# Rudrabha/Wav2Lip

Hardware: NVIDIA H100
Metric: 96x96 face-crops/sec (B=128, T=5, mel 80x16) (higher is better)
Workload: dtype f16

## Files before the change

wav2lip_b200/csrc/conv_igemm.cuh:

```cuda
#pragma once

#include <cuda.h>
#include <cuda_bf16.h>
#include <cuda_fp16.h>
#include <stdint.h>

#include "wgmma.cuh"

namespace w2l {

constexpr int kTileM = 128;
constexpr int kMaxTaps = 49;
constexpr int kMaxSteps = 3 * kMaxTaps;
constexpr int kSmemExtra = 2048;
constexpr int kSmemMax = 227 * 1024;

enum : int { ACT_NONE = 0, ACT_RELU = 1, ACT_LRELU = 2 };

struct EpiParams {
    int Wout, Hout, N;
    int act;
    int out_f32;
    void* out;
    long long out_sn, out_sy, out_sx;
// ... 72 lines not shown
        "cp.async.bulk.tensor.3d.shared::cluster.global.mbarrier::complete_tx::bytes [%0], [%1, {%3, %4, %5}], [%2];"
        ::"r"(dst), "l"(reinterpret_cast<uint64_t>(desc)), "r"(bar), "r"(c0), "r"(c1), "r"(c2)
        : "memory");
}
__device__ __forceinline__ void pdl_launch_dependents() { asm volatile("griddepcontrol.launch_dependents;" ::: "memory"); }
__device__ __forceinline__ void pdl_wait() { asm volatile("griddepcontrol.wait;" ::: "memory"); }

template <int BK>
__device__ __forceinline__ uint64_t make_kmajor_desc(uint32_t saddr) {
    return wg_desc(saddr, 16, 8 * BK * 2, BK * 2);
}

template <int BN, int BK, bool kBF16>
__device__ __forceinline__ void wg_mma_tile(float (&acc)[2][BN / 2], uint32_t a, uint32_t sbo_a, uint32_t b, bool accumulate) {
#pragma unroll
    for (int k = 0; k < BK / 16; ++k) {
        const uint64_t bd = make_kmajor_desc<BK>(b + 32u * k);
        const uint32_t on = (accumulate || k > 0) ? 1u : 0u;
        wgmma_m64k16<BN, kBF16>(acc[0], wg_desc(a + 32u * k, 16, sbo_a, BK * 2), bd, on, 0);
        wgmma_m64k16<BN, kBF16>(acc[1], wg_desc(a + 8u * sbo_a + 32u * k, 16, sbo_a, BK * 2), bd, on, 0);
    }
}

template <int BN, int BK, int MT = 1>
struct ConvCfg {
    static constexpr int kATile = kTileM * BK * 2;
    static constexpr int kABytes = MT * kATile;
    static constexpr int kBBytes = BN * BK * 2;
    static constexpr int kStageBytes = kABytes + kBBytes;
    static constexpr int kEW = BN < 64 ? BN : 64;
    static constexpr int kCW = BN < 32 ? BN : 32;
    static constexpr int kPasses = BN / kEW;
    static constexpr int kBoxBytes = kTileM * kEW * 2;
    static constexpr int kGrpRaw = kPasses * kBoxBytes > xbuf_bytes<kCW>() ? kPasses * kBoxBytes : xbuf_bytes<kCW>();
    static constexpr int kGrpBytes = (kGrpRaw + 1023) / 1024 * 1024;
    static constexpr int kStagesRaw = (kSmemMax - kSmemExtra - 2 * kGrpBytes) / kStageBytes;
    static constexpr int kStages = kStagesRaw > 8 ? 8 : kStagesRaw;
    static constexpr int kRingBytes = (kStages * kStageBytes + 1023) / 1024 * 1024;
    static constexpr int kSmemBytes = kRingBytes + 2 * kGrpBytes + kSmemExtra;
    static constexpr int kThreads = 384;
    static_assert(BN <= 128, "a warpgroup holds at most 128 fp32 accumulator columns per row");
    static_assert(kBoxBytes % 1024 == 0, "staging boxes must keep the 1024-byte swizzle alignment");
    static_assert(kStages >= 2, "need a pipeline");
    static_assert(kSmemBytes <= kSmemMax, "shared-memory carve-up exceeds the per-CTA limit");
};

__device__ int g_f16_overflow = 0;

template <bool kBF16>
__device__ __forceinline__ uint32_t pack2_live(float a, float b, uint32_t live_bits) {
    if constexpr (kBF16) {
        __nv_bfloat162 h = __floats2bfloat162_rn(a, b);
        return *reinterpret_cast<uint32_t*>(&h);
    } else {
        __half2 h = __floats2half2_rn(a, b);
        const uint32_t u = *reinterpret_cast<uint32_t*>(&h);
        if (((u & 0x7FFF7FFFu) + 0x04000400u) & live_bits) g_f16_overflow = 1;
        return u;
    }
}
template <bool kBF16>
__device__ __forceinline__ uint32_t pack2(float a, float b, bool live = true) {
    return pack2_live<kBF16>(a, b, live ? 0x80008000u : 0u);
}
// ... 81 lines not shown
                for (int j = 0; j < CH / 8; ++j) {
                    uint4 o;
                    o.x = pack2<kBF16>(f[8 * j + 0], f[8 * j + 1]);
                    o.y = pack2<kBF16>(f[8 * j + 2], f[8 * j + 3]);
                    o.z = pack2<kBF16>(f[8 * j + 4], f[8 * j + 5]);
                    o.w = pack2<kBF16>(f[8 * j + 6], f[8 * j + 7]);
                    op[j] = o;
                    if (e.x2) {
                        const float2 h0 = unpack2<kBF16>(o.x), h1 = unpack2<kBF16>(o.y);
                        const float2 h2 = unpack2<kBF16>(o.z), h3 = unpack2<kBF16>(o.w);
                        uint4 l;
                        l.x = pack2<kBF16>(f[8 * j + 0] - h0.x, f[8 * j + 1] - h0.y);
                        l.y = pack2<kBF16>(f[8 * j + 2] - h1.x, f[8 * j + 3] - h1.y);
                        l.z = pack2<kBF16>(f[8 * j + 4] - h2.x, f[8 * j + 5] - h2.y);
                        l.w = pack2<kBF16>(f[8 * j + 6] - h3.x, f[8 * j + 7] - h3.y);
                        op[(e.out_lo_off >> 3) + j] = l;
                    }
                }
            }
        }
    }
}

constexpr int kProducerRegs = 40, kConsumerRegs = 232;
template <int kRegs>
__device__ __forceinline__ void setmaxnreg_dec() { asm volatile("setmaxnreg.dec.sync.aligned.u32 %0;" ::"n"(kRegs)); }
template <int kRegs>
__device__ __forceinline__ void setmaxnreg_inc() { asm volatile("setmaxnreg.inc.sync.aligned.u32 %0;" ::"n"(kRegs)); }
__device__ __forceinline__ void named_bar_sync(uint32_t id, uint32_t n) { asm volatile("bar.sync %0, %1;" ::"r"(id), "r"(n) : "memory"); }
__device__ __forceinline__ void named_bar_arrive(uint32_t id, uint32_t n) { asm volatile("bar.arrive %0, %1;" ::"r"(id), "r"(n) : "memory"); }

template <int BN, int BK, bool kBF16, bool kHead, int MT = 1>
__global__ void __launch_bounds__(ConvCfg<BN, BK, MT>::kThreads, 1) conv_igemm_kernel(const __grid_constant__ ConvParams p) {
    pdl_launch_dependents();
    using Cfg = ConvCfg<BN, BK, MT>;
    constexpr int kStages = Cfg::kStages;
    static_assert(!kHead || BN == 32, "fused head expects the 32-channel output block");
    static_assert(MT == 1 || MT == 2, "one or two M tiles per unit");

    extern __shared__ uint8_t smem_raw[];
    const uint32_t smem_raw_u32 = smem_u32(smem_raw);
    const uint32_t smem_base = (smem_raw_u32 + 1023u) & ~1023u;
    const uint32_t grp_base = smem_base + Cfg::kRingBytes;
    const uint32_t bar_base = grp_base + 2 * Cfg::kGrpBytes;
    auto full_bar = [&](int s) { return bar_base + 8u * s; };
    auto empty_bar = [&](int s) { return bar_base + 8u * (kStages + s); };
    auto res_bar = [&](int g) { return bar_base + 8u * (2 * kStages + g); };

    const int warp = threadIdx.x >> 5;
    const int lane = threadIdx.x & 31;

    if (warp == 0 && lane == 0) {
        tma_prefetch_desc(&p.tmA);
        tma_prefetch_desc(&p.tmB);
        if (p.tma_epi) {
            tma_prefetch_desc(&p.tmO);
            tma_prefetch_desc(&p.tmR);
        }
    }
    if (warp == 1 && lane == 0) {
        for (int s = 0; s < kStages; ++s) {
            mbar_init(full_bar(s), 1);
            mbar_init(empty_bar(s), 4 * MT);
        }
        for (int g = 0; g < 2; ++g) mbar_init(res_bar(g), 1);
        fence_barrier_init();
    }
    __syncthreads();
    pdl_wait();

    const int m_tiles = p.tiles_x * p.tiles_y * p.tiles_n;
    const int m_units = (m_tiles + MT - 1) / MT;
    const int total_tiles = m_units * p.n_tiles;
    const int k_steps = p.ntaps * p.kc_per_tap;

    if (warp < 4) {
        setmaxnreg_dec<kProducerRegs>();
        if (warp == 0 && lane == 0) {
            int stage = 0;
            uint32_t phase = 0;
            for (int tile = blockIdx.x; tile < total_tiles; tile += gridDim.x) {
                const int nt = tile % p.n_tiles;
                const int mu = tile / p.n_tiles;
                int x_in0[MT], y_in0[MT], n0[MT];
#pragma unroll
                for (int mt = 0; mt < MT; ++mt) {
// ... 1 lines not shown
                    const int tx = m % p.tiles_x;
                    const int ty = (m / p.tiles_x) % p.tiles_y;
                    const int tn = m / (p.tiles_x * p.tiles_y);
                    x_in0[mt] = tx * p.bw * p.sx;
                    y_in0[mt] = ty * p.bh * p.sy;
                    n0[mt] = tn * p.bn;
                }
                for (int t = 0; t < p.ntaps; ++t) {
                    for (int kc = 0; kc < p.kc_per_tap; ++kc) {
                        mbar_wait(empty_bar(stage), phase ^ 1u);
                        const uint32_t a_dst = smem_base + stage * Cfg::kStageBytes;
                        const uint32_t b_dst = a_dst + Cfg::kABytes;
                        mbar_arrive_expect_tx(full_bar(stage), p.stage_tx_bytes);
#pragma unroll
                        for (int mt = 0; mt < MT; ++mt)
                            tma_load_4d(a_dst + mt * Cfg::kATile, &p.tmA, full_bar(stage), kc * BK + (p.a_lo[t] ? p.a_lo_off : 0),
                                        x_in0[mt] + p.dx[t], y_in0[mt] + p.dy[t], n0[mt]);
                        tma_load_3d(b_dst, &p.tmB, full_bar(stage), kc * BK, nt * BN, p.b_slab[t]);
                        if (++stage == kStages) { stage = 0; phase ^= 1u; }
                    }
                }
            }
        }
    } else {
        setmaxnreg_inc<kConsumerRegs>();
        const int g = (warp - 4) >> 2;
        const int q = (warp - 4) & 3;
        const int mt = MT == 2 ? g : 0;
        constexpr int kItStride = MT == 2 ? 1 : 2;
        const int it0 = MT == 2 ? 0 : g;
        const int rows_valid = p.bw * p.bh * p.bn;
        const uint32_t bar_id = 1 + g;
        const uint32_t my_turn = 3 + g, their_turn = 3 + (g ^ 1);
        const uint32_t grp = grp_base + g * Cfg::kGrpBytes;
        float acc[2][BN / 2];
        auto mainloop = [&](int s0, bool hand_off) {
            int stage = s0 % kStages;
            uint32_t phase = static_cast<uint32_t>(s0 / kStages) & 1u;
            int prev = -1;
            for (int ks = 0; ks < k_steps; ++ks) {
                mbar_wait(full_bar(stage), phase);
                const uint32_t a_addr = smem_base + stage * Cfg::kStageBytes + mt * Cfg::kATile;
                wg_fence();
                wg_mma_tile<BN, BK, kBF16>(acc, a_addr, 8 * BK * 2, smem_base + stage * Cfg::kStageBytes + Cfg::kABytes, ks > 0);
                wg_commit();
                wg_wait<1>();
// ... 128 lines not shown
```

wav2lip_b200/csrc/conv_patch.cuh:

```cuda
#pragma once

#include "conv_igemm.cuh"

namespace w2l {

constexpr int kPatchTileW = 8, kPatchTileH = 16;
constexpr int kChTileH = 32;
__host__ __device__ constexpr bool patch_chmajor(int BN, int BK, bool head) { return BN == 64 && BK == 64 && !head; }
constexpr int kPatchThreads = 384;
constexpr int kPatchMaxTaps = 9;
constexpr int kPatchMaxStages = 8;

struct alignas(64) PatchParams {
    CUtensorMap tmA;
    CUtensorMap tmB;
    CUtensorMap tmO;
    CUtensorMap tmO2;
    int has_out2;
    int tiles_x, tiles_y;
    int kc;
    int stages;
    int PW, PH;
    int ox, oy;
    int ntaps;
// ... 68 lines not shown
            for (int tile = blockIdx.x; tile < total_tiles; tile += gridDim.x) {
                const int n = tile / tiles_per_img;
                const int r = tile - n * tiles_per_img;
                const int ty = r / p.tiles_x, tx = r - ty * p.tiles_x;
                mbar_wait(empty_bar(stage), phase ^ 1u);
                mbar_arrive_expect_tx(full_bar(stage), static_cast<uint32_t>(kc) * p.patch_bytes);
                for (int c = 0; c < kc; ++c)
                    tma_load_4d(a_base + (stage * kc + c) * p.patch_stride, &p.tmA, full_bar(stage), c * BK,
                                tx * kPatchTileW + p.ox, ty * kTileH + p.oy, n);
                if (++stage == stages) { stage = 0; phase ^= 1u; }
            }
        }
    } else if constexpr (kCM) {
        setmaxnreg_inc<kConsumerRegs>();
        const int grp = (warp - 4) >> 2;
        const int q = (warp - 4) & 3;
        const int ch = 16 * q + (lane >> 2);
        const float sc0 = p.cscale[ch], sh0 = p.cshift[ch], sc1 = p.cscale[ch + 8], sh1 = p.cshift[ch + 8];
        const int px = 2 * (lane & 3);
        const EpiParams& e = p.ep;
        const uint32_t stg = stg_base + grp * kStgBytes;
        const bool leader = (q == 0 && lane == 0);
        const uint32_t bar_id = 1 + grp;
        const int lm_row = lane >> 4, lm_px = lane & 7;
        const uint32_t lm_chunk = 16u * (2 * q + ((lane >> 3) & 1));
        const uint32_t sbo_b = static_cast<uint32_t>(p.PW) * kRowBytes;
        uint32_t tap_off[kPatchMaxTaps];
#pragma unroll
        for (int t = 0; t < kPatchMaxTaps; ++t) tap_off[t] = (t < ntaps ? p.tap_row[t] : 0) * kRowBytes;
        mbar_wait(w_bar, 0);
        float acc[128];
        for (int it = grp;; it += 2) {
            const int tile = blockIdx.x + it * gridDim.x;
            if (tile >= total_tiles) break;
            const int stage = it % stages;
            const int n = tile / tiles_per_img;
            const int r = tile - n * tiles_per_img;
            const int ty = r / p.tiles_x, tx = r - ty * p.tiles_x;

            mbar_wait(full_bar(stage), static_cast<uint32_t>(it / stages) & 1u);
            wg_fence();
            for (int c = 0; c < kc; ++c) {
                const uint32_t patch = a_base + (stage * kc + c) * p.patch_stride;
#pragma unroll
                for (int tap = 0; tap < kPatchMaxTaps; ++tap)
                    if (tap < ntaps) {
#pragma unroll
                        for (int k = 0; k < BK / 16; ++k)
                            wgmma_m64k16<256, kBF16>(acc, make_kmajor_desc<BK>(w_base + (tap * kc + c) * kSlab + 32u * k),
                                                     wg_desc(patch + tap_off[tap] + 32u * k, 16, sbo_b, kRowBytes),
                                                     (c | tap | k) != 0 ? 1u : 0u, 0);
                    }
            }
            wg_commit();
            wg_wait<0>();
            wg_fence_regs<128>(acc);
            if (p.res_row < 0 && lane == 0) mbar_arrive(empty_bar(stage));

            const uint32_t res_base = a_base + stage * kc * p.patch_stride;
#pragma unroll
            for (int i = 0; i < 16; ++i) {
#pragma unroll
                for (int h = 0; h < 2; ++h) {
                    float* a = acc + 8 * i + 4 * h;
                    a[0] = fmaf(a[0], sc0, sh0); a[1] = fmaf(a[1], sc0, sh0);
                    a[2] = fmaf(a[2], sc1, sh1); a[3] = fmaf(a[3], sc1, sh1);
                }
                if (p.res_row >= 0) {
                    uint32_t ad = res_base + static_cast<uint32_t>(p.res_row + (2 * i + lm_row) * p.PW + lm_px) * kRowBytes + lm_chunk;
                    ad ^= ((ad >> 7) & 7u) << 4;
                    uint32_t rv[4];
                    asm volatile("ldmatrix.sync.aligned.m8n8.x4.trans.shared.b16 {%0,%1,%2,%3}, [%4];"
                                 : "=r"(rv[0]), "=r"(rv[1]), "=r"(rv[2]), "=r"(rv[3]) : "r"(ad));
#pragma unroll
                    for (int m = 0; m < 4; ++m) {
                        const float2 v = unpack2<kBF16>(rv[m]);
                        acc[8 * i + 2 * m] += v.x;
                        acc[8 * i + 2 * m + 1] += v.y;
                    }
                }
            }
            if (p.res_row >= 0) {
                __syncwarp();
                if (lane == 0) mbar_arrive(empty_bar(stage));
            }
            if (e.act == ACT_RELU) {
#pragma unroll
                for (int j = 0; j < 128; ++j) acc[j] = fmaxf(acc[j], 0.0f);
            } else if (e.act == ACT_LRELU) {
#pragma unroll
                for (int j = 0; j < 128; ++j) acc[j] = acc[j] > 0.0f ? acc[j] : 0.01f * acc[j];
            }
            const int x = tx * kPatchTileW + px;
            const uint32_t live_x = (x < e.Wout ? 0x8000u : 0u) | (x + 1 < e.Wout ? 0x80000000u : 0u);
            const int rows_live = e.Hout - ty * kTileH;
            if (leader) asm volatile("cp.async.bulk.wait_group.read 0;" ::: "memory");
            named_bar_sync(bar_id, 128);
#pragma unroll
            for (int i = 0; i < 16; ++i) {
                uint32_t ad = stg + static_cast<uint32_t>((2 * i + lm_row) * kPatchTileW + lm_px) * kRowBytes + lm_chunk;
                ad ^= ((ad >> 7) & 7u) << 4;
                const uint32_t l0 = 2 * i < rows_live ? live_x : 0u, l1 = 2 * i + 1 < rows_live ? live_x : 0u;
                const uint32_t o0 = pack2_live<kBF16>(acc[8 * i + 0], acc[8 * i + 1], l0);
                const uint32_t o1 = pack2_live<kBF16>(acc[8 * i + 2], acc[8 * i + 3], l0);
                const uint32_t o2 = pack2_live<kBF16>(acc[8 * i + 4], acc[8 * i + 5], l1);
                const uint32_t o3 = pack2_live<kBF16>(acc[8 * i + 6], acc[8 * i + 7], l1);
                asm volatile("stmatrix.sync.aligned.m8n8.x4.trans.shared.b16 [%0], {%1,%2,%3,%4};"
                             ::"r"(ad), "r"(o0), "r"(o1), "r"(o2), "r"(o3) : "memory");
            }
            asm volatile("fence.proxy.async.shared::cta;" ::: "memory");
            named_bar_sync(bar_id, 128);
            if (leader) {
                asm volatile("cp.async.bulk.tensor.4d.global.shared::cta.bulk_group [%0, {%2, %3, %4, %5}], [%1];"
                             ::"l"(reinterpret_cast<uint64_t>(&p.tmO)), "r"(stg), "r"(0), "r"(tx * kPatchTileW), "r"(ty * kTileH), "r"(n)
                             : "memory");
                asm volatile("cp.async.bulk.commit_group;" ::: "memory");
            }
        }
        if (leader) asm volatile("cp.async.bulk.wait_group 0;" ::: "memory");
    } else {
        const int grp = (warp - 4) >> 2;
        const int q = (warp - 4) & 3;
        const int row = q * 32 + lane;
        const int py = row >> 3, px = row & 7;
        const EpiParams& e = p.ep;
        constexpr uint32_t kOutRow = BN * 2;
        constexpr uint32_t kOutSwz = (kOutRow == 128) ? 7u : (kOutRow == 64) ? 3u : 1u;
        constexpr uint32_t kInSwz = (BK == 64) ? 7u : (BK == 32) ? 3u : 1u;
        const uint32_t stg = stg_base + grp * kStgBytes;
        float* const xb = reinterpret_cast<float*>(smem_raw + (xb_base - smem_raw_u32) + grp * xbuf_bytes<32>());
        const bool leader = (q == 0 && lane == 0);
        const uint32_t bar_id = 1 + grp;
        const uint32_t sbo_a = static_cast<uint32_t>(p.PW) * kRowBytes;
        uint32_t tap_off[kPatchMaxTaps];
#pragma unroll
        for (int t = 0; t < kPatchMaxTaps; ++t) tap_off[t] = (t < ntaps ? p.tap_row[t] : 0) * kRowBytes;
        mbar_wait(w_bar, 0);
        float acc[2][BN / 2];
        for (int it = grp;; it += 2) {
            const int tile = blockIdx.x + it * gridDim.x;
// ... 100 lines not shown
```

wav2lip_b200/csrc/host_launch.cuh:

```cuda
#pragma once

typedef void (*ConvKernelFn)(const ConvParams);
struct ConvKernelEntry { int BN, BK; bool bf16, head; ConvKernelFn fn; int smem; uint64_t attr_set; int mt; int threads; };

#define W2L_CONV_ENTRY(BN_, BK_)                                                                                                        \
    {BN_, BK_, false, false, conv_igemm_kernel<BN_, BK_, false, false>, ConvCfg<BN_, BK_>::kSmemBytes, 0, 1, ConvCfg<BN_, BK_>::kThreads}, \
    {BN_, BK_, true, false, conv_igemm_kernel<BN_, BK_, true, false>, ConvCfg<BN_, BK_>::kSmemBytes, 0, 1, ConvCfg<BN_, BK_>::kThreads}
#define W2L_CONV_ENTRY_MT2(BN_, BK_)                                                                                                    \
    {BN_, BK_, false, false, conv_igemm_kernel<BN_, BK_, false, false, 2>, ConvCfg<BN_, BK_, 2>::kSmemBytes, 0, 2, ConvCfg<BN_, BK_, 2>::kThreads}, \
    {BN_, BK_, true, false, conv_igemm_kernel<BN_, BK_, true, false, 2>, ConvCfg<BN_, BK_, 2>::kSmemBytes, 0, 2, ConvCfg<BN_, BK_, 2>::kThreads}

static ConvKernelEntry g_conv_kernels[] = {
    W2L_CONV_ENTRY(16, 16), W2L_CONV_ENTRY(16, 32), W2L_CONV_ENTRY(16, 64),
    W2L_CONV_ENTRY(32, 16), W2L_CONV_ENTRY(32, 32), W2L_CONV_ENTRY(32, 64),
    W2L_CONV_ENTRY(64, 16), W2L_CONV_ENTRY(64, 32), W2L_CONV_ENTRY(64, 64),
    W2L_CONV_ENTRY(128, 16), W2L_CONV_ENTRY(128, 32), W2L_CONV_ENTRY(128, 64),
    W2L_CONV_ENTRY_MT2(64, 64), W2L_CONV_ENTRY_MT2(64, 32),
    {32, 16, false, true, conv_igemm_kernel<32, 16, false, true>, ConvCfg<32, 16>::kSmemBytes, 0, 1, ConvCfg<32, 16>::kThreads},
    {32, 16, true, true, conv_igemm_kernel<32, 16, true, true>, ConvCfg<32, 16>::kSmemBytes, 0, 1, ConvCfg<32, 16>::kThreads},
};

static ConvKernelEntry* find_conv_kernel(int BN, int BK, bool bf16, bool head, int mt = 1) {
    for (auto& e : g_conv_kernels)
        if (e.BN == BN && e.BK == BK && e.bf16 == bf16 && e.head == head && e.mt == mt) return &e;
    return nullptr;
}

typedef void (*PatchKernelFn)(const PatchParams);
struct PatchKernelEntry { int BN, BK; bool bf16, head; PatchKernelFn fn; uint64_t attr_set; };
#define W2L_PATCH_ENTRY(BN_, BK_)                                                    \
    {BN_, BK_, false, false, conv_patch_kernel<BN_, BK_, false, false>, 0},    \
    {BN_, BK_, true, false, conv_patch_kernel<BN_, BK_, true, false>, 0}
static PatchKernelEntry g_patch_kernels[] = {
    W2L_PATCH_ENTRY(16, 16), W2L_PATCH_ENTRY(16, 32), W2L_PATCH_ENTRY(16, 64),
    W2L_PATCH_ENTRY(32, 16), W2L_PATCH_ENTRY(32, 32), W2L_PATCH_ENTRY(32, 64),
    W2L_PATCH_ENTRY(64, 16), W2L_PATCH_ENTRY(64, 32), W2L_PATCH_ENTRY(64, 64),
    {32, 16, false, true, conv_patch_kernel<32, 16, false, true>, 0},
    {32, 16, true, true, conv_patch_kernel<32, 16, true, true>, 0},
};
static PatchKernelEntry* find_patch_kernel(int BN, int BK, bool bf16, bool head) {
    for (auto& e : g_patch_kernels)
        if (e.BN == BN && e.BK == BK && e.bf16 == bf16 && e.head == head) return &e;
    return nullptr;
}

typedef void (*CtKernelFn)(const ConvTParams);
struct CtKernelEntry { int BK; bool bf16; CtKernelFn fn; uint64_t attr_set; };
// ... 36 lines not shown
    k->fold = op.fold ? 1 : 0;
    k->m_tiles = op.m_tiles; k->n_tiles = op.n_tiles; k->grid = op.grid;
}

static int launch_conv(w2l_ctx* ctx, const Op& op, cudaStream_t st, bool pdl = true) {
    pdl = pdl && ctx->use_pdl;
    if (op.ctf) {
        CtKernelEntry* e = nullptr;
        for (auto& k : g_ct_kernels) if (k.BK == op.BK && k.bf16 == ctx->bf16) e = &k;
        if (!e) return fail(W2L_EINVAL, "no fused convT kernel for BK=%d", op.BK);
        CKR(ensure_smem_attr(&e->attr_set, ctx->device, (const void*)e->fn, kCtSmemMax));
        CK(launch_k(e->fn, op.grid, kCtThreads, op.dyn_smem, st, op.tp, pdl));
        ctx->launches++;
        return W2L_OK;
    }
    if (op.patch) {
        PatchKernelEntry* e = find_patch_kernel(op.BN, op.BK, ctx->bf16, op.head);
        if (!e) return fail(W2L_EINVAL, "no patch kernel for BN=%d BK=%d head=%d", op.BN, op.BK, (int)op.head);
        CKR(ensure_smem_attr(&e->attr_set, ctx->device, (const void*)e->fn, kSmemMax));
        CK(launch_k(e->fn, op.grid, kPatchThreads, op.dyn_smem, st, op.pp, pdl));
        ctx->launches++;
        return W2L_OK;
    }
    ConvKernelEntry* e = find_conv_kernel(op.BN, op.BK, ctx->bf16, op.head, op.MT);
    if (!e) return fail(W2L_EINVAL, "no conv kernel for BN=%d BK=%d head=%d MT=%d", op.BN, op.BK, (int)op.head, op.MT);
    CKR(ensure_smem_attr(&e->attr_set, ctx->device, (const void*)e->fn, e->smem));
    CK(launch_k(e->fn, op.grid, e->threads, (size_t)e->smem, st, op.cp, pdl));
    ctx->launches++;
    return W2L_OK;
}
```

wav2lip_b200/csrc/host_ops.cuh:

```cuda
#pragma once

static int pick_bk(int cin_pad) { return (cin_pad % 64 == 0) ? 64 : (cin_pad % 32 == 0) ? 32 : 16; }
static int round_up(int a, int b) { return (a + b - 1) / b * b; }

static void pick_box(int W, int H, int N, int sx, int sy, int* bw, int* bh, int* bn) {
    double best = 1e30;
    int b_w = 1, b_h = 1, b_n = 1;
    for (int w = 1; w <= std::min(W, kTileM); ++w) {
        if (w * sx > 256) break;
        for (int h = 1; h <= std::min(H, kTileM / w); ++h) {
            if (h * sy > 256) break;
            int n = std::min(kTileM / (w * h), std::max(N, 1));
            if (n < 1) continue;
            if (n > 256) n = 256;
            const double tiles = (double)((W + w - 1) / w) * ((H + h - 1) / h) * ((N + n - 1) / n);
            const double cost = tiles - 1e-6 * w - 1e-9 * h;
            if (cost < best) { best = cost; b_w = w; b_h = h; b_n = n; }
        }
    }
    *bw = b_w; *bh = b_h; *bn = b_n;
}

struct ConvArgs {
    std::string name;
    Act in, out;
    const PackedW* w = nullptr;
    int sx = 1, sy = 1;
    int Hl = 0, Wl = 0;
    int osy = 1, osx = 1;
    int phy = 0, phx = 0;
    const Act* res = nullptr;
    const float* scale = nullptr;
    const float* shift = nullptr;
    int ch_off = 0;
    int act = ACT_RELU;
// ... 156 lines not shown
        CK(cudaMemcpy(h.chead_b, a.head_b, 3 * 4, cudaMemcpyDeviceToHost));
    }
    const long long total = (long long)h.tiles_x * h.tiles_y * a.in.N;
    op.grid = (int)std::min<long long>(total, ctx->num_sms);
    op.fold = w.fold; op.m_tiles = (int)total; op.n_tiles = 1;
    op.flops = 2.0 * a.macs_per_pixel * (double)a.Wl * a.Hl * a.in.N;
    pl->ops.push_back(op);
    return W2L_OK;
}

static int make_conv_op(w2l_ctx* ctx, Plan* pl, const ConvArgs& a) {
    if (!get_encode_fn()) return fail(W2L_ENODEV, "cuTensorMapEncodeTiled is not available (no CUDA driver?)");
    const PackedW& w = *a.w;
    if (a.in.C != w.cin_pad) return fail(W2L_EINVAL, "%s: input view has %d channels, weights packed for %d", a.name.c_str(), a.in.C, w.cin_pad);
    if (a.cout % 16 != 0) return fail(W2L_EINVAL, "%s: cout %d not a multiple of 16", a.name.c_str(), a.cout);
    PatchGeom geom;
    if (patch_eligible(ctx, a, &geom)) return make_patch_op(ctx, pl, a, geom);
    Op op;
    op.type = OP_CONV;
    op.name = a.name + (w.fold ? " [fold]" : "");
    const int BK = pick_bk(w.cin_pad);
    int bw, bh, bn;
    pick_box(a.Wl, a.Hl, a.in.N, a.sx, a.sy, &bw, &bh, &bn);
    const int tiles_x = (a.Wl + bw - 1) / bw, tiles_y = (a.Hl + bh - 1) / bh, tiles_n = (a.in.N + bn - 1) / bn;
    const int m_tiles = tiles_x * tiles_y * tiles_n;
    int BN = 16;
    for (int cand : {128, 64, 32, 16})
        if (a.cout % cand == 0) { BN = cand; break; }
    if (a.head) BN = 32;
    else
        while (BN > 32 && m_tiles * (a.cout / BN) < ctx->num_sms && a.cout % (BN / 2) == 0) BN /= 2;
    if (w.cout_pad % BN != 0) return fail(W2L_EINVAL, "%s: cout_pad %d vs BN %d", a.name.c_str(), w.cout_pad, BN);
    op.BN = BN; op.BK = BK; op.head = a.head;
    const int n_tiles_ = a.cout / BN;
    if (ctx->use_mt2 && !a.head && find_conv_kernel(BN, BK, ctx->bf16, false, 2) &&
        (long long)((m_tiles + 1) / 2) * n_tiles_ >= 2LL * ctx->num_sms)
        op.MT = 2;
    if (op.MT == 2) op.name += " [2M]";

    ConvParams& p = op.cp;
    memset(&p, 0, sizeof(p));
    CKR(encode_act_map(ctx, &p.tmA, a.in, BK, bw * a.sx, bh * a.sy, bn, a.sx, a.sy, a.name.c_str()));
    CKR(encode_w_map(ctx, &p.tmB, w, BK, BN, a.name.c_str()));
    p.tiles_x = tiles_x; p.tiles_y = tiles_y; p.tiles_n = tiles_n; p.n_tiles = a.cout / BN;
    p.bw = bw; p.bh = bh; p.bn = bn;
    p.sx = a.sx; p.sy = a.sy;
    p.ntaps = w.ntaps; p.kc_per_tap = w.cin_pad / BK;
    p.stage_tx_bytes = (unsigned)(op.MT * bw * bh * bn * BK * 2 + BN * BK * 2);
    fill_epi(&p.ep, a);
    p.tma_epi = 0;
    if (ctx->use_tma_epi && !ctx->x2 && !a.head && !a.out.f32) {
        EncodeTiledFn enc = get_encode_fn();
        const int EW = BN < 64 ? BN : 64;
        const CUtensorMapDataType dt = ctx->bf16 ? CU_TENSOR_MAP_DATA_TYPE_BFLOAT16 : CU_TENSOR_MAP_DATA_TYPE_FLOAT16;
        const CUtensorMapSwizzle esw = EW == 64 ? CU_TENSOR_MAP_SWIZZLE_128B : EW == 32 ? CU_TENSOR_MAP_SWIZZLE_64B : CU_TENSOR_MAP_SWIZZLE_32B;
        cuuint64_t dims[4] = {(cuuint64_t)std::min(a.cout, a.out.C), (cuuint64_t)a.Wl, (cuuint64_t)a.Hl, (cuuint64_t)a.in.N};
        cuuint32_t box[4] = {(cuuint32_t)EW, (cuuint32_t)bw, (cuuint32_t)bh, (cuuint32_t)bn};
        cuuint32_t es[4] = {1, 1, 1, 1};
// ... 155 lines not shown
```

wav2lip_b200/csrc/host_types.h:

```cpp
#pragma once

static thread_local std::string g_err;

static int fail(int code, const char* fmt, ...) {
    char buf[1024];
    va_list ap;
    va_start(ap, fmt);
    vsnprintf(buf, sizeof(buf), fmt, ap);
    va_end(ap);
    g_err = buf;
    return code;
}

#define CK(call)                                                                                         \
    do {                                                                                                 \
        cudaError_t e_ = (call);                                                                         \
        if (e_ != cudaSuccess)                                                                           \
            return fail(W2L_ECUDA, "%s failed: %s (%s:%d)", #call, cudaGetErrorString(e_), __FILE__, __LINE__); \
    } while (0)
#define CKR(expr)               \
    do {                        \
        int r_ = (expr);        \
        if (r_ != W2L_OK) return r_; \
    } while (0)
// ... 108 lines not shown
    float* scale = nullptr;
    float* shift = nullptr;
    std::vector<DevMem<>> mem;
    int n_scale = 0;
    bool gemm_convT = false;
    bool has_all_taps = false;
    bool loaded = false;
};

struct NetW {
    std::vector<LayerW> layers;
    DevMem<float> head_w;
    DevMem<float> head_b;
    bool loaded = false;
};

enum OpType { OP_CONV = 0, OP_INGEST = 1, OP_L2NORM = 2, OP_DISC_HEAD = 3, OP_MAXPOOL = 4, OP_CHAN_L2NORM = 5, OP_S3FD_EXPORT = 6 };

struct Op {
    int type = OP_CONV;
    std::string name;
    ConvParams cp;
    int BN = 0, BK = 0, MT = 1;
    bool head = false;
    int grid = 0;
    double flops = 0;
    bool patch = false;
    PatchParams pp;
    int dyn_smem = 0;
    bool ctf = false;
    ConvTParams tp;
    bool fold = false;
    int m_tiles = 0, n_tiles = 0;
    IngestParams ip;
    int ingest_src = 0;
    const void* aux_in = nullptr;
    int aux_rows = 0, aux_dim = 0;
    int aux_out = 0;
    int aux_pitch = 0, aux_lo = 0;
    const uint16_t* sp_in = nullptr; uint16_t* sp_out = nullptr; const float* sp_f32 = nullptr; const float* sp_w = nullptr;
    int sp_N = 0, sp_H = 0, sp_W = 0, sp_C = 0, sp_Cout = 0, sp_maxout = 0;
    int lane = 0;
    bool join_side = false;
};

struct S3fdDetWork {
// ... 115 lines not shown
```

wav2lip_b200/csrc/w2l_api.cu:

```cuda
#include <cuda.h>
#include <cuda_runtime.h>

#include <algorithm>
#include <cmath>
#include <cstdarg>
#include <cstdio>
#include <cstdint>
#include <cstdlib>
#include <cstring>
#include <dlfcn.h>
#include <functional>
#include <initializer_list>
#include <map>
#include <memory>
#include <string>
#include <vector>

#include "../../include/w2l.h"
#include "aux_kernels.cuh"
#include "conv_igemm.cuh"
#include "conv_patch.cuh"
#include "convt_fused.cuh"
#include "mel.cuh"
#include "netspec.h"
// ... 581 lines not shown
    for (const Op& op : pl.ops)
        if (op.type == OP_CONV) { ctx->last_block_kernels.emplace_back(); op_kernel_info(ctx, op, &ctx->last_block_kernels.back()); }
    Plan* lp = ctx->last_plan[W2L_NET_DISC];
    const int r = run_plan(ctx, &pl, x, nullptr, nullptr, nullptr, st);
    ctx->last_plan[W2L_NET_DISC] = lp;
    CKR(r);
    const long long total = (long long)N * L.cout * Ho * Wo;
    const int blocks = (int)std::min<long long>((total + 255) / 256, ctx->num_sms * 16);
    if (ctx->bf16) export_kernel<true><<<blocks, 256, 0, st>>>(out.base, y, N, Ho, Wo, L.cout, out.Cs, 0, out.lo_off);
    else export_kernel<false><<<blocks, 256, 0, st>>>(out.base, y, N, Ho, Wo, L.cout, out.Cs, 0, out.lo_off);
    ctx->launches++;
    CK(cudaStreamSynchronize(st));
    return W2L_OK;
}

int w2l_debug_kernel_table(int cap, w2l_kernel_info* out) {
    std::vector<w2l_kernel_info> t;
    auto add = [&](int fam, int bn, int bk, int mt, bool head, bool bf16) {
        w2l_kernel_info k;
        memset(&k, 0, sizeof(k));
        k.family = fam; k.bn = bn; k.bk = bk; k.mt = mt; k.head = head ? 1 : 0; k.bf16 = bf16 ? 1 : 0;
        t.push_back(k);
    };
    for (const auto& e : g_conv_kernels) add(W2L_KFAM_IGEMM, e.BN, e.BK, e.mt, e.head, e.bf16);
    for (const auto& e : g_patch_kernels) add(W2L_KFAM_PATCH, e.BN, e.BK, 1, e.head, e.bf16);
    for (const auto& e : g_ct_kernels) add(W2L_KFAM_CONVT_FUSED, kCtBN, e.BK, 1, false, e.bf16);
    if (!out) return (int)t.size();
    const int k = std::min<int>(std::max(cap, 0), (int)t.size());
    for (int i = 0; i < k; ++i) out[i] = t[i];
    return k;
}

int w2l_debug_plan_kernels(w2l_ctx* ctx, int net, int cap, w2l_kernel_info* out) {
    if (!ctx || net < -1 || net > 3) return fail(W2L_EINVAL, "bad argument");
    std::vector<w2l_kernel_info> t;
    if (net < 0) {
        t = ctx->last_block_kernels;
    } else {
        const Plan* pl = ctx->last_plan[net];
        if (!pl) return fail(W2L_ESTATE, "no forward has run for net %d", net);
        for (const Op& op : pl->ops)
            if (op.type == OP_CONV) { t.emplace_back(); op_kernel_info(ctx, op, &t.back()); }
    }
    if (!out) return (int)t.size();
    const int k = std::min<int>(std::max(cap, 0), (int)t.size());
    for (int i = 0; i < k; ++i) out[i] = t[i];
    return k;
// ... 630 lines not shown
```

Before: 54720.

## Add channel-major 256-pixel igemm variant for deep 128-channel convolutions

Adds a channel-major form of the implicit-GEMM conv kernel. Each consumer warpgroup computes 64 output channels by 256 pixels with a single wgmma of N=256, using the weights as the A operand and the activation box as B. This doubles the pixel tile and reuses each weight tile across more pixels, lowering per-tile overhead on deep layers. The patch kernel's epilogue is factored into a shared helper that the new path also uses. The host picks the variant only when the conv has enough K steps, 128-channel output, no stride on the output, and a tile fill close to the regular path, so it risks worse load balance or tail effects on some layers.

```diff
diff --git a/wav2lip_b200/csrc/conv_igemm.cuh b/wav2lip_b200/csrc/conv_igemm.cuh
--- a/wav2lip_b200/csrc/conv_igemm.cuh
+++ b/wav2lip_b200/csrc/conv_igemm.cuh
@@ -118,17 +118,19 @@
     }
 }
 
-template <int BN, int BK, int MT = 1>
+constexpr int kCmPixels = 256;
+template <int BN, int BK, int MT = 1, bool kCM = false>
 struct ConvCfg {
-    static constexpr int kATile = kTileM * BK * 2;
+    static constexpr int kRowsA = kCM ? kCmPixels : kTileM;
+    static constexpr int kATile = kRowsA * BK * 2;
     static constexpr int kABytes = MT * kATile;
     static constexpr int kBBytes = BN * BK * 2;
     static constexpr int kStageBytes = kABytes + kBBytes;
     static constexpr int kEW = BN < 64 ? BN : 64;
     static constexpr int kCW = BN < 32 ? BN : 32;
-    static constexpr int kPasses = BN / kEW;
-    static constexpr int kBoxBytes = kTileM * kEW * 2;
-    static constexpr int kGrpRaw = kPasses * kBoxBytes > xbuf_bytes<kCW>() ? kPasses * kBoxBytes : xbuf_bytes<kCW>();
+    static constexpr int kPasses = kCM ? 1 : BN / kEW;
+    static constexpr int kBoxBytes = kRowsA * kEW * 2;
+    static constexpr int kGrpRaw = (kCM || kPasses * kBoxBytes > xbuf_bytes<kCW>()) ? kPasses * kBoxBytes : xbuf_bytes<kCW>();
     static constexpr int kGrpBytes = (kGrpRaw + 1023) / 1024 * 1024;
     static constexpr int kStagesRaw = (kSmemMax - kSmemExtra - 2 * kGrpBytes) / kStageBytes;
     static constexpr int kStages = kStagesRaw > 8 ? 8 : kStagesRaw;
@@ -136,6 +138,7 @@
     static constexpr int kSmemBytes = kRingBytes + 2 * kGrpBytes + kSmemExtra;
     static constexpr int kThreads = 384;
     static_assert(BN <= 128, "a warpgroup holds at most 128 fp32 accumulator columns per row");
+    static_assert(!kCM || (BN == 128 && BK == 64 && MT == 1), "channel-major form: 128 channels, 128-byte K rows, one tile");
     static_assert(kBoxBytes % 1024 == 0, "staging boxes must keep the 1024-byte swizzle alignment");
     static_assert(kStages >= 2, "need a pipeline");
     static_assert(kSmemBytes <= kSmemMax, "shared-memory carve-up exceeds the per-CTA limit");
@@ -263,21 +266,86 @@
     }
 }
 
+__device__ __forceinline__ void named_bar_sync(uint32_t id, uint32_t n) { asm volatile("bar.sync %0, %1;" ::"r"(id), "r"(n) : "memory"); }
+__device__ __forceinline__ void named_bar_arrive(uint32_t id, uint32_t n) { asm volatile("bar.arrive %0, %1;" ::"r"(id), "r"(n) : "memory"); }
+
+template <bool kBF16, typename AfterRes, typename Live>
+__device__ __forceinline__ void chmajor_epilogue(float (&acc)[128], float sc0, float sh0, float sc1, float sh1, int act,
+                                                 uint32_t res, int res_pitch, AfterRes&& after_res, Live&& live, uint32_t stg,
+                                                 uint32_t bar_id, bool leader, const CUtensorMap* tmO, int c0, int c1, int c2,
+                                                 int c3) {
+    constexpr uint32_t kRowB = 128;
+    const int lane = threadIdx.x & 31, q = (threadIdx.x >> 5) & 3;
+    const int lm_row = lane >> 4, lm_px = lane & 7;
+    const uint32_t lm_chunk = 16u * (2 * q + ((lane >> 3) & 1));
+#pragma unroll
+    for (int i = 0; i < 16; ++i) {
+#pragma unroll
+        for (int h = 0; h < 2; ++h) {
+            float* a = acc + 8 * i + 4 * h;
+            a[0] = fmaf(a[0], sc0, sh0); a[1] = fmaf(a[1], sc0, sh0);
+            a[2] = fmaf(a[2], sc1, sh1); a[3] = fmaf(a[3], sc1, sh1);
+        }
+        if (res != 0) {
+            uint32_t ad = res + static_cast<uint32_t>((2 * i + lm_row) * res_pitch + lm_px) * kRowB + lm_chunk;
+            ad ^= ((ad >> 7) & 7u) << 4;
+            uint32_t rv[4];
+            asm volatile("ldmatrix.sync.aligned.m8n8.x4.trans.shared.b16 {%0,%1,%2,%3}, [%4];"
+                         : "=r"(rv[0]), "=r"(rv[1]), "=r"(rv[2]), "=r"(rv[3]) : "r"(ad));
+#pragma unroll
+            for (int m = 0; m < 4; ++m) {
+                const float2 v = unpack2<kBF16>(rv[m]);
+                acc[8 * i + 2 * m] += v.x;
+                acc[8 * i + 2 * m + 1] += v.y;
+            }
+        }
+    }
+    after_res();
+    if (act == ACT_RELU) {
+#pragma unroll
+        for (int j = 0; j < 128; ++j) acc[j] = fmaxf(acc[j], 0.0f);
+    } else if (act == ACT_LRELU) {
+#pragma unroll
+        for (int j = 0; j < 128; ++j) acc[j] = acc[j] > 0.0f ? acc[j] : 0.01f * acc[j];
+    }
+    if (leader) asm volatile("cp.async.bulk.wait_group.read 0;" ::: "memory");
+    named_bar_sync(bar_id, 128);
+#pragma unroll
+    for (int i = 0; i < 16; ++i) {
+        uint32_t ad = stg + static_cast<uint32_t>((2 * i + lm_row) * 8 + lm_px) * kRowB + lm_chunk;
+        ad ^= ((ad >> 7) & 7u) << 4;
+        const uint32_t l0 = live(2 * i), l1 = live(2 * i + 1);
+        const uint32_t o0 = pack2_live<kBF16>(acc[8 * i + 0], acc[8 * i + 1], l0);
+        const uint32_t o1 = pack2_live<kBF16>(acc[8 * i + 2], acc[8 * i + 3], l0);
+        const uint32_t o2 = pack2_live<kBF16>(acc[8 * i + 4], acc[8 * i + 5], l1);
+        const uint32_t o3 = pack2_live<kBF16>(acc[8 * i + 6], acc[8 * i + 7], l1);
+        asm volatile("stmatrix.sync.aligned.m8n8.x4.trans.shared.b16 [%0], {%1,%2,%3,%4};"
+                     ::"r"(ad), "r"(o0), "r"(o1), "r"(o2), "r"(o3) : "memory");
+    }
+    asm volatile("fence.proxy.async.shared::cta;" ::: "memory");
+    named_bar_sync(bar_id, 128);
+    if (leader) {
+        asm volatile("cp.async.bulk.tensor.4d.global.shared::cta.bulk_group [%0, {%2, %3, %4, %5}], [%1];"
+                     ::"l"(reinterpret_cast<uint64_t>(tmO)), "r"(stg), "r"(c0), "r"(c1), "r"(c2), "r"(c3)
+                     : "memory");
+        asm volatile("cp.async.bulk.commit_group;" ::: "memory");
+    }
+}
+
 constexpr int kProducerRegs = 40, kConsumerRegs = 232;
 template <int kRegs>
 __device__ __forceinline__ void setmaxnreg_dec() { asm volatile("setmaxnreg.dec.sync.aligned.u32 %0;" ::"n"(kRegs)); }
 template <int kRegs>
 __device__ __forceinline__ void setmaxnreg_inc() { asm volatile("setmaxnreg.inc.sync.aligned.u32 %0;" ::"n"(kRegs)); }
-__device__ __forceinline__ void named_bar_sync(uint32_t id, uint32_t n) { asm volatile("bar.sync %0, %1;" ::"r"(id), "r"(n) : "memory"); }
-__device__ __forceinline__ void named_bar_arrive(uint32_t id, uint32_t n) { asm volatile("bar.arrive %0, %1;" ::"r"(id), "r"(n) : "memory"); }
-
-template <int BN, int BK, bool kBF16, bool kHead, int MT = 1>
-__global__ void __launch_bounds__(ConvCfg<BN, BK, MT>::kThreads, 1) conv_igemm_kernel(const __grid_constant__ ConvParams p) {
+
+template <int BN, int BK, bool kBF16, bool kHead, int MT = 1, bool kCM = false>
+__global__ void __launch_bounds__(ConvCfg<BN, BK, MT, kCM>::kThreads, 1) conv_igemm_kernel(const __grid_constant__ ConvParams p) {
     pdl_launch_dependents();
-    using Cfg = ConvCfg<BN, BK, MT>;
+    using Cfg = ConvCfg<BN, BK, MT, kCM>;
     constexpr int kStages = Cfg::kStages;
     static_assert(!kHead || BN == 32, "fused head expects the 32-channel output block");
     static_assert(MT == 1 || MT == 2, "one or two M tiles per unit");
+    static_assert(!kCM || !kHead, "the channel-major form stages its epilogue");
 
     extern __shared__ uint8_t smem_raw[];
     const uint32_t smem_raw_u32 = smem_u32(smem_raw);
@@ -302,7 +370,7 @@
     if (warp == 1 && lane == 0) {
         for (int s = 0; s < kStages; ++s) {
             mbar_init(full_bar(s), 1);
-            mbar_init(empty_bar(s), 4 * MT);
+            mbar_init(empty_bar(s), kCM ? 8 : 4 * MT);
         }
         for (int g = 0; g < 2; ++g) mbar_init(res_bar(g), 1);
         fence_barrier_init();
@@ -350,6 +418,87 @@
                 }
             }
         }
+    } else if constexpr (kCM) {
+        setmaxnreg_inc<kConsumerRegs>();
+        const int g = (warp - 4) >> 2;
+        const int q = (warp - 4) & 3;
+        const uint32_t bar_id = 1 + g;
+        const bool leader = (q == 0 && lane == 0);
+        const uint32_t stg = grp_base + g * Cfg::kGrpBytes;
+        const bool has_res = p.ep.res != nullptr;
+        const int rows_valid = p.bw * p.bh * p.bn;
+        const int ch = 64 * g + 16 * q + (lane >> 2);
+        auto tile_origin = [&](int tile_, int* nt_, int* x0_, int* y0_, int* n0_) {
+            *nt_ = tile_ % p.n_tiles;
+            const int m_ = tile_ / p.n_tiles;
+            *x0_ = (m_ % p.tiles_x) * p.bw;
+            *y0_ = ((m_ / p.tiles_x) % p.tiles_y) * p.bh;
+            *n0_ = (m_ / (p.tiles_x * p.tiles_y)) * p.bn;
+        };
+        auto fetch_res = [&](int tile_) {
+            int nt_, x0_, y0_, n0_;
+            tile_origin(tile_, &nt_, &x0_, &y0_, &n0_);
+            mbar_arrive_expect_tx(res_bar(g), p.epi_box_bytes);
+            tma_load_4d(stg, &p.tmR, res_bar(g), nt_ * BN + 64 * g, x0_, y0_, n0_);
+        };
+        if (has_res && leader && static_cast<int>(blockIdx.x) < total_tiles) fetch_res(blockIdx.x);
+        float acc[128];
+        int stage = 0;
+        uint32_t phase = 0, rphase = 0;
+        for (int tile = blockIdx.x; tile < total_tiles; tile += gridDim.x) {
+            int prev = -1;
+            for (int ks = 0; ks < k_steps; ++ks) {
+                mbar_wait(full_bar(stage), phase);
+                const uint32_t box = smem_base + stage * Cfg::kStageBytes;
+                const uint32_t wts = box + Cfg::kABytes + g * (64 * BK * 2);
+                wg_fence();
+#pragma unroll
+                for (int k = 0; k < BK / 16; ++k)
+                    wgmma_m64k16<256, kBF16>(acc, make_kmajor_desc<BK>(wts + 32u * k), make_kmajor_desc<BK>(box + 32u * k),
+                                             (ks | k) != 0 ? 1u : 0u, 0);
+                wg_commit();
+                wg_wait<1>();
+                if (prev >= 0 && lane == 0) mbar_arrive(empty_bar(prev));
+                prev = stage;
+                if (++stage == kStages) { stage = 0; phase ^= 1u; }
+            }
+            wg_wait<0>();
+            wg_fence_regs<128>(acc);
+            if (lane == 0) mbar_arrive(empty_bar(prev));
+
+            int nt, x0, y0, n0;
+            tile_origin(tile, &nt, &x0, &y0, &n0);
+            uint64_t live = ~0ull;
+            if constexpr (!kBF16) {
+                const int xr = p.ep.Wout - x0, yr = p.ep.Hout - y0, nr = p.ep.N - n0;
+                if (rows_valid < kCmPixels || xr < p.bw || yr < p.bh || nr < p.bn) {
+                    live = 0;
+#pragma unroll 1
+                    for (int b = 0; b < 64; ++b) {
+                        const int px = 8 * (b >> 1) + 2 * (lane & 3) + (b & 1);
+                        const int xx = px % p.bw, yy = (px / p.bw) % p.bh, nn = px / (p.bw * p.bh);
+                        if (px < rows_valid && xx < xr && yy < yr && nn < nr) live |= 1ull << b;
+                    }
+                }
+            }
+            if (has_res) {
+                mbar_wait(res_bar(g), rphase);
+                rphase ^= 1u;
+            }
+            const float* const sc = p.ep.scale + nt * BN + ch;
+            const float* const sh = p.ep.shift + nt * BN + ch;
+            chmajor_epilogue<kBF16>(
+                acc, __ldg(sc), __ldg(sh), __ldg(sc + 8), __ldg(sh + 8), p.ep.act, has_res ? stg : 0u, 8, [] {},
+                [&](int j) {
+                    return (static_cast<uint32_t>(live >> (2 * j)) & 1u) << 15 | (static_cast<uint32_t>(live >> (2 * j + 1)) & 1u) << 31;
+                },
+                stg, bar_id, leader, &p.tmO, nt * BN + 64 * g, x0, y0, n0);
+            if (has_res && leader && tile + static_cast<int>(gridDim.x) < total_tiles) {
+                asm volatile("cp.async.bulk.wait_group.read 0;" ::: "memory");
+                fetch_res(tile + gridDim.x);
+            }
+        }
+        if (leader) asm volatile("cp.async.bulk.wait_group 0;" ::: "memory");
     } else {
         setmaxnreg_inc<kConsumerRegs>();
         const int g = (warp - 4) >> 2;
diff --git a/wav2lip_b200/csrc/conv_patch.cuh b/wav2lip_b200/csrc/conv_patch.cuh
--- a/wav2lip_b200/csrc/conv_patch.cuh
+++ b/wav2lip_b200/csrc/conv_patch.cuh
@@ -114,8 +114,6 @@
         const uint32_t stg = stg_base + grp * kStgBytes;
         const bool leader = (q == 0 && lane == 0);
         const uint32_t bar_id = 1 + grp;
-        const int lm_row = lane >> 4, lm_px = lane & 7;
-        const uint32_t lm_chunk = 16u * (2 * q + ((lane >> 3) & 1));
         const uint32_t sbo_b = static_cast<uint32_t>(p.PW) * kRowBytes;
         uint32_t tap_off[kPatchMaxTaps];
 #pragma unroll
@@ -149,65 +147,20 @@
             wg_fence_regs<128>(acc);
             if (p.res_row < 0 && lane == 0) mbar_arrive(empty_bar(stage));
 
-            const uint32_t res_base = a_base + stage * kc * p.patch_stride;
-#pragma unroll
-            for (int i = 0; i < 16; ++i) {
-#pragma unroll
-                for (int h = 0; h < 2; ++h) {
-                    float* a = acc + 8 * i + 4 * h;
-                    a[0] = fmaf(a[0], sc0, sh0); a[1] = fmaf(a[1], sc0, sh0);
-                    a[2] = fmaf(a[2], sc1, sh1); a[3] = fmaf(a[3], sc1, sh1);
-                }
-                if (p.res_row >= 0) {
-                    uint32_t ad = res_base + static_cast<uint32_t>(p.res_row + (2 * i + lm_row) * p.PW + lm_px) * kRowBytes + lm_chunk;
-                    ad ^= ((ad >> 7) & 7u) << 4;
-                    uint32_t rv[4];
-                    asm volatile("ldmatrix.sync.aligned.m8n8.x4.trans.shared.b16 {%0,%1,%2,%3}, [%4];"
-                                 : "=r"(rv[0]), "=r"(rv[1]), "=r"(rv[2]), "=r"(rv[3]) : "r"(ad));
-#pragma unroll
-                    for (int m = 0; m < 4; ++m) {
-                        const float2 v = unpack2<kBF16>(rv[m]);
-                        acc[8 * i + 2 * m] += v.x;
-                        acc[8 * i + 2 * m + 1] += v.y;
-                    }
-                }
-            }
-            if (p.res_row >= 0) {
-                __syncwarp();
-                if (lane == 0) mbar_arrive(empty_bar(stage));
-            }
-            if (e.act == ACT_RELU) {
-#pragma unroll
-                for (int j = 0; j < 128; ++j) acc[j] = fmaxf(acc[j], 0.0f);
-            } else if (e.act == ACT_LRELU) {
-#pragma unroll
-                for (int j = 0; j < 128; ++j) acc[j] = acc[j] > 0.0f ? acc[j] : 0.01f * acc[j];
-            }
             const int x = tx * kPatchTileW + px;
             const uint32_t live_x = (x < e.Wout ? 0x8000u : 0u) | (x + 1 < e.Wout ? 0x80000000u : 0u);
             const int rows_live = e.Hout - ty * kTileH;
-            if (leader) asm volatile("cp.async.bulk.wait_group.read 0;" ::: "memory");
-            named_bar_sync(bar_id, 128);
-#pragma unroll
-            for (int i = 0; i < 16; ++i) {
-                uint32_t ad = stg + static_cast<uint32_t>((2 * i + lm_row) * kPatchTileW + lm_px) * kRowBytes + lm_chunk;
-                ad ^= ((ad >> 7) & 7u) << 4;
-                const uint32_t l0 = 2 * i < rows_live ? live_x : 0u, l1 = 2 * i + 1 < rows_live ? live_x : 0u;
-                const uint32_t o0 = pack2_live<kBF16>(acc[8 * i + 0], acc[8 * i + 1], l0);
-                const uint32_t o1 = pack2_live<kBF16>(acc[8 * i + 2], acc[8 * i + 3], l0);
-                const uint32_t o2 = pack2_live<kBF16>(acc[8 * i + 4], acc[8 * i + 5], l1);
-                const uint32_t o3 = pack2_live<kBF16>(acc[8 * i + 6], acc[8 * i + 7], l1);
-                asm volatile("stmatrix.sync.aligned.m8n8.x4.trans.shared.b16 [%0], {%1,%2,%3,%4};"
-                             ::"r"(ad), "r"(o0), "r"(o1), "r"(o2), "r"(o3) : "memory");
-            }
-            asm volatile("fence.proxy.async.shared::cta;" ::: "memory");
-            named_bar_sync(bar_id, 128);
-            if (leader) {
-                asm volatile("cp.async.bulk.tensor.4d.global.shared::cta.bulk_group [%0, {%2, %3, %4, %5}], [%1];"
-                             ::"l"(reinterpret_cast<uint64_t>(&p.tmO)), "r"(stg), "r"(0), "r"(tx * kPatchTileW), "r"(ty * kTileH), "r"(n)
-                             : "memory");
-                asm volatile("cp.async.bulk.commit_group;" ::: "memory");
-            }
+            const uint32_t res = p.res_row >= 0 ? a_base + (stage * kc * p.patch_stride + p.res_row * kRowBytes) : 0u;
+            chmajor_epilogue<kBF16>(
+                acc, sc0, sh0, sc1, sh1, e.act, res, p.PW,
+                [&] {
+                    if (p.res_row >= 0) {
+                        __syncwarp();
+                        if (lane == 0) mbar_arrive(empty_bar(stage));
+                    }
+                },
+                [&](int j) { return j < rows_live ? live_x : 0u; }, stg, bar_id, leader, &p.tmO, 0, tx * kPatchTileW,
+                ty * kTileH, n);
         }
         if (leader) asm volatile("cp.async.bulk.wait_group 0;" ::: "memory");
     } else {
diff --git a/wav2lip_b200/csrc/host_launch.cuh b/wav2lip_b200/csrc/host_launch.cuh
--- a/wav2lip_b200/csrc/host_launch.cuh
+++ b/wav2lip_b200/csrc/host_launch.cuh
@@ -1,14 +1,17 @@
 #pragma once
 
 typedef void (*ConvKernelFn)(const ConvParams);
-struct ConvKernelEntry { int BN, BK; bool bf16, head; ConvKernelFn fn; int smem; uint64_t attr_set; int mt; int threads; };
+struct ConvKernelEntry { int BN, BK; bool bf16, head; ConvKernelFn fn; int smem; uint64_t attr_set; int mt; int threads; bool cm; };
 
 #define W2L_CONV_ENTRY(BN_, BK_)                                                                                                        \
-    {BN_, BK_, false, false, conv_igemm_kernel<BN_, BK_, false, false>, ConvCfg<BN_, BK_>::kSmemBytes, 0, 1, ConvCfg<BN_, BK_>::kThreads}, \
-    {BN_, BK_, true, false, conv_igemm_kernel<BN_, BK_, true, false>, ConvCfg<BN_, BK_>::kSmemBytes, 0, 1, ConvCfg<BN_, BK_>::kThreads}
+    {BN_, BK_, false, false, conv_igemm_kernel<BN_, BK_, false, false>, ConvCfg<BN_, BK_>::kSmemBytes, 0, 1, ConvCfg<BN_, BK_>::kThreads, false}, \
+    {BN_, BK_, true, false, conv_igemm_kernel<BN_, BK_, true, false>, ConvCfg<BN_, BK_>::kSmemBytes, 0, 1, ConvCfg<BN_, BK_>::kThreads, false}
 #define W2L_CONV_ENTRY_MT2(BN_, BK_)                                                                                                    \
-    {BN_, BK_, false, false, conv_igemm_kernel<BN_, BK_, false, false, 2>, ConvCfg<BN_, BK_, 2>::kSmemBytes, 0, 2, ConvCfg<BN_, BK_, 2>::kThreads}, \
-    {BN_, BK_, true, false, conv_igemm_kernel<BN_, BK_, true, false, 2>, ConvCfg<BN_, BK_, 2>::kSmemBytes, 0, 2, ConvCfg<BN_, BK_, 2>::kThreads}
+    {BN_, BK_, false, false, conv_igemm_kernel<BN_, BK_, false, false, 2>, ConvCfg<BN_, BK_, 2>::kSmemBytes, 0, 2, ConvCfg<BN_, BK_, 2>::kThreads, false}, \
+    {BN_, BK_, true, false, conv_igemm_kernel<BN_, BK_, true, false, 2>, ConvCfg<BN_, BK_, 2>::kSmemBytes, 0, 2, ConvCfg<BN_, BK_, 2>::kThreads, false}
+#define W2L_CONV_ENTRY_CM(BN_, BK_)                                                                                                     \
+    {BN_, BK_, false, false, conv_igemm_kernel<BN_, BK_, false, false, 1, true>, ConvCfg<BN_, BK_, 1, true>::kSmemBytes, 0, 1, ConvCfg<BN_, BK_, 1, true>::kThreads, true}, \
+    {BN_, BK_, true, false, conv_igemm_kernel<BN_, BK_, true, false, 1, true>, ConvCfg<BN_, BK_, 1, true>::kSmemBytes, 0, 1, ConvCfg<BN_, BK_, 1, true>::kThreads, true}
 
 static ConvKernelEntry g_conv_kernels[] = {
     W2L_CONV_ENTRY(16, 16), W2L_CONV_ENTRY(16, 32), W2L_CONV_ENTRY(16, 64),
@@ -16,13 +19,14 @@
     W2L_CONV_ENTRY(64, 16), W2L_CONV_ENTRY(64, 32), W2L_CONV_ENTRY(64, 64),
     W2L_CONV_ENTRY(128, 16), W2L_CONV_ENTRY(128, 32), W2L_CONV_ENTRY(128, 64),
     W2L_CONV_ENTRY_MT2(64, 64), W2L_CONV_ENTRY_MT2(64, 32),
-    {32, 16, false, true, conv_igemm_kernel<32, 16, false, true>, ConvCfg<32, 16>::kSmemBytes, 0, 1, ConvCfg<32, 16>::kThreads},
-    {32, 16, true, true, conv_igemm_kernel<32, 16, true, true>, ConvCfg<32, 16>::kSmemBytes, 0, 1, ConvCfg<32, 16>::kThreads},
+    W2L_CONV_ENTRY_CM(128, 64),
+    {32, 16, false, true, conv_igemm_kernel<32, 16, false, true>, ConvCfg<32, 16>::kSmemBytes, 0, 1, ConvCfg<32, 16>::kThreads, false},
+    {32, 16, true, true, conv_igemm_kernel<32, 16, true, true>, ConvCfg<32, 16>::kSmemBytes, 0, 1, ConvCfg<32, 16>::kThreads, false},
 };
 
-static ConvKernelEntry* find_conv_kernel(int BN, int BK, bool bf16, bool head, int mt = 1) {
+static ConvKernelEntry* find_conv_kernel(int BN, int BK, bool bf16, bool head, int mt = 1, bool cm = false) {
     for (auto& e : g_conv_kernels)
-        if (e.BN == BN && e.BK == BK && e.bf16 == bf16 && e.head == head && e.mt == mt) return &e;
+        if (e.BN == BN && e.BK == BK && e.bf16 == bf16 && e.head == head && e.mt == mt && e.cm == cm) return &e;
     return nullptr;
 }
 
@@ -105,8 +109,8 @@
         ctx->launches++;
         return W2L_OK;
     }
-    ConvKernelEntry* e = find_conv_kernel(op.BN, op.BK, ctx->bf16, op.head, op.MT);
-    if (!e) return fail(W2L_EINVAL, "no conv kernel for BN=%d BK=%d head=%d MT=%d", op.BN, op.BK, (int)op.head, op.MT);
+    ConvKernelEntry* e = find_conv_kernel(op.BN, op.BK, ctx->bf16, op.head, op.MT, op.cm);
+    if (!e) return fail(W2L_EINVAL, "no conv kernel for BN=%d BK=%d head=%d MT=%d cm=%d", op.BN, op.BK, (int)op.head, op.MT, (int)op.cm);
     CKR(ensure_smem_attr(&e->attr_set, ctx->device, (const void*)e->fn, e->smem));
     CK(launch_k(e->fn, op.grid, e->threads, (size_t)e->smem, st, op.cp, pdl));
     ctx->launches++;
diff --git a/wav2lip_b200/csrc/host_ops.cuh b/wav2lip_b200/csrc/host_ops.cuh
--- a/wav2lip_b200/csrc/host_ops.cuh
+++ b/wav2lip_b200/csrc/host_ops.cuh
@@ -2,15 +2,18 @@
 
 static int pick_bk(int cin_pad) { return (cin_pad % 64 == 0) ? 64 : (cin_pad % 32 == 0) ? 32 : 16; }
 static int round_up(int a, int b) { return (a + b - 1) / b * b; }
-
-static void pick_box(int W, int H, int N, int sx, int sy, int* bw, int* bh, int* bn) {
+constexpr int kCmMinSteps = 18;
+constexpr int kCmMinCtaSteps = 48;
+constexpr double kCmFillMargin = 0.06;
+
+static void pick_box(int W, int H, int N, int sx, int sy, int* bw, int* bh, int* bn, int pixels = kTileM) {
     double best = 1e30;
     int b_w = 1, b_h = 1, b_n = 1;
-    for (int w = 1; w <= std::min(W, kTileM); ++w) {
+    for (int w = 1; w <= std::min(W, pixels); ++w) {
         if (w * sx > 256) break;
-        for (int h = 1; h <= std::min(H, kTileM / w); ++h) {
+        for (int h = 1; h <= std::min(H, pixels / w); ++h) {
             if (h * sy > 256) break;
-            int n = std::min(kTileM / (w * h), std::max(N, 1));
+            int n = std::min(pixels / (w * h), std::max(N, 1));
             if (n < 1) continue;
             if (n > 256) n = 256;
             const double tiles = (double)((W + w - 1) / w) * ((H + h - 1) / h) * ((N + n - 1) / n);
@@ -213,18 +216,39 @@
     const int BK = pick_bk(w.cin_pad);
     int bw, bh, bn;
     pick_box(a.Wl, a.Hl, a.in.N, a.sx, a.sy, &bw, &bh, &bn);
-    const int tiles_x = (a.Wl + bw - 1) / bw, tiles_y = (a.Hl + bh - 1) / bh, tiles_n = (a.in.N + bn - 1) / bn;
-    const int m_tiles = tiles_x * tiles_y * tiles_n;
+    int tiles_x = (a.Wl + bw - 1) / bw, tiles_y = (a.Hl + bh - 1) / bh, tiles_n = (a.in.N + bn - 1) / bn;
+    int m_tiles = tiles_x * tiles_y * tiles_n;
     int BN = 16;
     for (int cand : {128, 64, 32, 16})
         if (a.cout % cand == 0) { BN = cand; break; }
     if (a.head) BN = 32;
     else
         while (BN > 32 && m_tiles * (a.cout / BN) < ctx->num_sms && a.cout % (BN / 2) == 0) BN /= 2;
+    const int k_steps = w.ntaps * (w.cin_pad / BK);
+    if (ctx->use_tma_epi && !ctx->x2 && !a.head && !a.out.f32 && a.cout % 128 == 0 && w.cout_pad % 128 == 0 && BK == 64 &&
+        a.osx == 1 && a.osy == 1 && k_steps >= kCmMinSteps) {
+        int cw, ch, cn;
+        pick_box(a.Wl, a.Hl, a.in.N, a.sx, a.sy, &cw, &ch, &cn, kCmPixels);
+        const long long cm_tiles = (long long)((a.Wl + cw - 1) / cw) * ((a.Hl + ch - 1) / ch) * ((a.in.N + cn - 1) / cn);
+        const int S = ctx->num_sms, nt = a.cout / 128;
+        auto fill = [&](long long tiles, int pixels) {
+            const long long rounds = (tiles * nt + S - 1) / S;
+            return (double)a.Wl * a.Hl * a.in.N / ((double)rounds * S * pixels / nt);
+        };
+        if ((cm_tiles * nt + S - 1) / S * k_steps >= kCmMinCtaSteps &&
+            fill(cm_tiles, kCmPixels) >= (1.0 - kCmFillMargin) * fill(m_tiles, kTileM)) {
+            op.cm = true;
+            op.name += " [cm]";
+            BN = 128;
+            bw = cw; bh = ch; bn = cn;
+            tiles_x = (a.Wl + bw - 1) / bw; tiles_y = (a.Hl + bh - 1) / bh; tiles_n = (a.in.N + bn - 1) / bn;
+            m_tiles = tiles_x * tiles_y * tiles_n;
+        }
+    }
     if (w.cout_pad % BN != 0) return fail(W2L_EINVAL, "%s: cout_pad %d vs BN %d", a.name.c_str(), w.cout_pad, BN);
     op.BN = BN; op.BK = BK; op.head = a.head;
     const int n_tiles_ = a.cout / BN;
-    if (ctx->use_mt2 && !a.head && find_conv_kernel(BN, BK, ctx->bf16, false, 2) &&
+    if (ctx->use_mt2 && !a.head && !op.cm && find_conv_kernel(BN, BK, ctx->bf16, false, 2) &&
         (long long)((m_tiles + 1) / 2) * n_tiles_ >= 2LL * ctx->num_sms)
         op.MT = 2;
     if (op.MT == 2) op.name += " [2M]";
diff --git a/wav2lip_b200/csrc/host_types.h b/wav2lip_b200/csrc/host_types.h
--- a/wav2lip_b200/csrc/host_types.h
+++ b/wav2lip_b200/csrc/host_types.h
@@ -154,6 +154,7 @@
     std::string name;
     ConvParams cp;
     int BN = 0, BK = 0, MT = 1;
+    bool cm = false;
     bool head = false;
     int grid = 0;
     double flops = 0;
diff --git a/wav2lip_b200/csrc/w2l_api.cu b/wav2lip_b200/csrc/w2l_api.cu
--- a/wav2lip_b200/csrc/w2l_api.cu
+++ b/wav2lip_b200/csrc/w2l_api.cu
@@ -627,7 +627,14 @@
         k.family = fam; k.bn = bn; k.bk = bk; k.mt = mt; k.head = head ? 1 : 0; k.bf16 = bf16 ? 1 : 0;
         t.push_back(k);
     };
-    for (const auto& e : g_conv_kernels) add(W2L_KFAM_IGEMM, e.BN, e.BK, e.mt, e.head, e.bf16);
+    for (const auto& e : g_conv_kernels)
+        if (!e.cm) add(W2L_KFAM_IGEMM, e.BN, e.BK, e.mt, e.head, e.bf16);
+    for (const auto& e : g_conv_kernels)
+        if (e.cm)
+            for (auto& k : t)
+                if (k.family == W2L_KFAM_IGEMM && k.bn == e.BN && k.bk == e.BK && k.mt == e.mt && k.head == (e.head ? 1 : 0) &&
+                    k.bf16 == (e.bf16 ? 1 : 0))
+                    snprintf(k.name, sizeof(k.name), "[cm]");
     for (const auto& e : g_patch_kernels) add(W2L_KFAM_PATCH, e.BN, e.BK, 1, e.head, e.bf16);
     for (const auto& e : g_ct_kernels) add(W2L_KFAM_CONVT_FUSED, kCtBN, e.BK, 1, false, e.bf16);
     if (!out) return (int)t.size();
```

Measured after the change: 58350, median of 6. 1.07x the previous value.
